# ZKTLabs/zkt-plonk

Measured on AMD Instinct MI355X. Metric: proofs/sec (withdraw, n=2^20), higher is better.
Workload: dtype u32 limbs (256-bit Montgomery); 1 GPU; full prove, WithdrawCircuit INPUTS=8 HEIGHT=64 Poseidon x5 (1019498 gates, 538 Poseidon gadgets), bn254, n=2^20, TABLE_SIZE=1024, 12 public inputs; parallelism=proofs sharded across 1 GPU(s), chained=True, distinct_witnesses=2, witness_on_device=True, table_cached=True, proof_bytes=802

## Files before the change

### zkt-plonk_amd/csrc/msm.hip

```cpp
#include "ctx.hpp"
#include "ec.hpp"
#include "ecx.hpp"
#include "hostec.hpp"
#include "msm.hpp"

#include <algorithm>
#include <functional>
#include <type_traits>
#include <cstdlib>
#include <cstring>

namespace zkt {

template <class C>
__global__ void k_srs_generate(Affine<typename C::Fq>* out, size_t count, Fe<typename C::Fr> tau_mont,
                               Affine<typename C::Fq> g, size_t first) {
    using Q = typename C::Fq;
    using R = typename C::Fr;
    size_t i = (size_t)blockIdx.x * blockDim.x + threadIdx.x;
    if (i >= count) return;
    Fe<R> s = fe_from_mont<R>(fe_from_mont<R>(fe_pow_u64<R>(tau_mont, (uint64_t)(first + i))));
    Xyzz<Q> acc = xyzz_identity<Q>();
    bool started = false;
#pragma unroll 1
// ... 194 lines not shown
    const bool in = threadIdx.x < 256;
    uint32_t incl = in ? mine : 0u;
#pragma unroll
    for (int d = 1; d < 64; d <<= 1) {
        const uint32_t o = __shfl_up(incl, d);
        if ((int)(threadIdx.x & 63) >= d) incl += o;
    }
    __syncthreads();
    if (in && (threadIdx.x & 63) == 63) wsum[threadIdx.x >> 6] = incl;
    __syncthreads();
    uint32_t before = 0;
    for (uint32_t w = 0; w < (threadIdx.x >> 6) && w < 4; ++w) before += wsum[w];
    return before + incl - (in ? mine : 0u);
}

template <class C, int DIG, bool VB = false>
__global__ __launch_bounds__(1024) void k_msm_bin_count(MsmBatch bt, int mont,
                                                        MsmWindows win, uint32_t per_block, uint32_t nb1, uint32_t lb,
                                                        uint32_t* counts) {
    using R = typename C::Fr;
    const uint32_t y = blockIdx.y;
    const Fe<R>* scalars = (const Fe<R>*)bt.scalars[y];
    const size_t n = bt.n[y];
    counts += y * bt.s_bin_offs;
    extern __shared__ uint32_t lds[];
    uint32_t* hist = lds;
    for (uint32_t b = threadIdx.x; b < nb1; b += 1024) hist[b] = 0;
    __syncthreads();
    Fe<R> sc[2];
    bool have[2];
#pragma unroll
    for (int t = 0; t < 2; ++t) {
        const uint32_t k = threadIdx.x + 1024u * t;
        const size_t i = (size_t)blockIdx.x * per_block + k;
        have[t] = k < per_block && i < n;
        if (have[t]) sc[t] = fe_load<R>(scalars + i);
    }
#pragma unroll
    for (int t = 0; t < 2; ++t) {
        if (!have[t]) continue;
        Fe<R> s = sc[t];
        if (VB) {
            if (mont) s = fe_from_mont<R>(s);
        } else if (!mont) {
            s = fe_to_mont<R>(s);
        }
        msm_for_each_digit_sel<R, DIG>(s, win, [&](int w, uint32_t d, uint32_t) {
            if (d) atomicAdd(&hist[(VB ? (uint32_t)w * bt.vb_stride + d : d) >> lb], 1u);
        });
    }
    __syncthreads();
    for (uint32_t b = threadIdx.x; b < nb1; b += 1024) counts[(size_t)b * gridDim.x + blockIdx.x] = hist[b];
}

constexpr int MSM_SCAN_TILE = 4096;
__global__ __launch_bounds__(1024) void k_msm_scan_tiles(uint32_t* counts, uint32_t total, uint32_t* aux, MsmBatch bt) {
    __shared__ uint32_t wsum[16];
    counts += blockIdx.y * bt.s_bin_offs;
    aux += blockIdx.y * bt.s_bin_aux;
    const uint32_t i0 = blockIdx.x * MSM_SCAN_TILE + threadIdx.x * 4;
    uint32_t v[4];
#pragma unroll
    for (int k = 0; k < 4; ++k) v[k] = (i0 + k < total) ? counts[i0 + k] : 0u;
    const uint32_t mine = v[0] + v[1] + v[2] + v[3];
    uint32_t all;
    uint32_t run = block_excl_scan_1024(mine, wsum, &all);
#pragma unroll
    for (int k = 0; k < 4; ++k) {
        if (i0 + k < total) counts[i0 + k] = run;
        run += v[k];
    }
    if (threadIdx.x == 0) aux[blockIdx.x] = all;
}
ZKT_D uint32_t msm_bin_off(const uint32_t* offs, const uint32_t* aux, size_t i, size_t total) {
    return (i < total) ? offs[i] + aux[i / MSM_SCAN_TILE] : aux[(total + MSM_SCAN_TILE - 1) / MSM_SCAN_TILE];
}
__global__ __launch_bounds__(1024) void k_msm_scan_aux(const uint32_t* offs, uint32_t* aux, uint32_t nt, uint32_t nblk,
                                                       uint32_t nb1, uint32_t* bin_start, uint32_t* tile_start,
                                                       uint2* tile_desc, uint32_t acc_threads, uint32_t B, uint32_t lanes_fold,
                                                       MsmBatch bt) {
    __shared__ uint32_t wsum[16];
    const uint32_t y = blockIdx.y;
    offs += y * bt.s_bin_offs;
    aux += y * bt.s_bin_aux;
    bin_start += y * bt.s_bin;
    tile_start += y * bt.s_bin;
    tile_desc += y * bt.s_tile_desc;
    uint32_t* heavy_count = bt.heavy[y];
    uint32_t* params = bt.params[y];
    uint32_t carry = 0;
    for (uint32_t base = 0; base < nt; base += 1024) {
        const uint32_t i = base + threadIdx.x;
        const uint32_t mine = (i < nt) ? aux[i] : 0u;
        uint32_t all;
        const uint32_t ex = block_excl_scan_1024(mine, wsum, &all);
        if (i < nt) aux[i] = carry + ex;
        carry += all;
    }
    if (threadIdx.x == 0) {
        aux[nt] = carry;
        *heavy_count = 0;
        uint32_t lo = 1;
        const uint32_t twice = lanes_fold ? (carry / B) / 11u : 2u * (carry / B);
        while (lo < (uint32_t)MSM_CHUNK_MIN && (lo + 1) * (lo + 1) <= twice) ++lo;
        const uint32_t even = (uint32_t)(((uint64_t)carry + acc_threads - 1) / acc_threads);
        params[0] = even > lo ? even : lo;
        params[1] = carry;
    }
    __syncthreads();
    const size_t total = (size_t)nb1 * nblk;
    uint32_t s = 0, tiles = 0;
    if (threadIdx.x <= nb1) s = msm_bin_off(offs, aux, (size_t)threadIdx.x * nblk, total);
    if (threadIdx.x < nb1) {
        const uint32_t e = msm_bin_off(offs, aux, (size_t)(threadIdx.x + 1) * nblk, total);
        tiles = (e - s + MSM_L2_TILE - 1) / MSM_L2_TILE;
    }
    uint32_t all;
    const uint32_t ex = block_excl_scan_1024(tiles, wsum, &all);
    if (threadIdx.x <= nb1) {
        bin_start[threadIdx.x] = s;
        tile_start[threadIdx.x] = ex;
    }
    if (threadIdx.x < nb1) {
        const uint32_t be = msm_bin_off(offs, aux, (size_t)(threadIdx.x + 1) * nblk, total);
        for (uint32_t k = 0; k < tiles; ++k) {
            const uint32_t ts = s + k * MSM_L2_TILE;
            tile_desc[ex + k] = make_uint2(ts, (ts + MSM_L2_TILE < be) ? ts + MSM_L2_TILE : be);
        }
    }
}

template <class C, class PF, int DIG, bool VB = false>
__global__ __launch_bounds__(1024) void k_msm_bin_scatter(MsmBatch bt, int mont,
                                                          MsmWindows win, uint32_t per_block,
                                                          uint32_t nb1, uint32_t lb, const uint32_t* offs,
                                                          const uint32_t* aux, typename PF::type* pairs) {
    using R = typename C::Fr;
    const uint32_t y = blockIdx.y;
    const Fe<R>* scalars = (const Fe<R>*)bt.scalars[y];
    const size_t n = bt.n[y], base_off = bt.base_off[y], count = bt.tcount[y];
    offs += y * bt.s_bin_offs;
    aux += y * bt.s_bin_aux;
    pairs = reinterpret_cast<typename PF::type*>(reinterpret_cast<char*>(pairs) + y * bt.s_pairs_bytes);
    extern __shared__ uint32_t lds[];
    __shared__ uint32_t wsum[16];
    uint32_t* cursor = lds;
    uint32_t* delta = lds + nb1;
    uint32_t* first = lds + 2 * nb1;
    typename PF::type* stage = (typename PF::type*)(lds + ((3 * nb1 + 3) & ~3u));
    const size_t total = (size_t)nb1 * gridDim.x;
    uint32_t g0 = 0, mine = 0;
    if (threadIdx.x < nb1) {
        const size_t at = (size_t)threadIdx.x * gridDim.x + blockIdx.x;
        g0 = msm_bin_off(offs, aux, at, total);
        mine = msm_bin_off(offs, aux, at + 1, total) - g0;
    }
    uint32_t staged;
    const uint32_t ex = block_excl_scan_1024(mine, wsum, &staged);
    if (threadIdx.x < nb1) {
        cursor[threadIdx.x] = ex;
        first[threadIdx.x] = ex;
        delta[threadIdx.x] = g0 - ex;
    }
    __syncthreads();
    Fe<R> sc[2];
    bool have[2];
#pragma unroll
    for (int t = 0; t < 2; ++t) {
        const uint32_t k = threadIdx.x + 1024u * t;
        const size_t i = (size_t)blockIdx.x * per_block + k;
// ... 15 lines not shown
                const uint32_t key = VB ? (uint32_t)w * bt.vb_stride + d : d;
                const uint32_t at = atomicAdd(&cursor[key >> lb], 1u);
                stage[at] = PF::make(key, VB ? (uint32_t)(base_off + i) : (uint32_t)((size_t)w * count + base_off + i), neg, lb);
            }
        });
    }
    __syncthreads();
    const uint32_t lane = threadIdx.x & 63u;
    for (uint32_t b = threadIdx.x >> 6; b < nb1; b += 16) {
        const uint32_t s0 = first[b], e0 = cursor[b], d = delta[b];
        for (uint32_t j = s0 + lane; j < e0; j += 64) pairs[d + j] = stage[j];
    }
}

struct L2Item {
    uint32_t s, e;
    bool valid;
};
ZKT_D L2Item msm_l2_item(uint32_t item, uint32_t nb1, const uint32_t* tile_start, const uint2* tile_desc) {
    L2Item r;
    r.valid = item < tile_start[nb1];
    r.s = 0; r.e = 0;
    if (!r.valid) return r;
    const uint2 d = tile_desc[item];
    r.s = d.x;
    r.e = d.y;
    return r;
}

template <class PF, int LC>
__global__ __launch_bounds__(256) void k_msm_l2_count(const typename PF::type* pairs, uint32_t nb1, uint32_t lb,
                                                      const uint32_t* tile_start, const uint2* tile_desc, uint32_t* cnt2,
                                                      MsmBatch bt) {
    constexpr uint32_t COLS = 1u << LC;
    {
        const uint32_t y = blockIdx.y;
        pairs = reinterpret_cast<const typename PF::type*>(reinterpret_cast<const char*>(pairs) + y * bt.s_pairs_bytes);
        tile_start += y * bt.s_bin;
        tile_desc += y * bt.s_tile_desc;
        cnt2 += y * bt.s_cnt;
    }
    __shared__ uint32_t hist[COLS];
    const L2Item it = msm_l2_item(blockIdx.x, nb1, tile_start, tile_desc);
    if (!it.valid) return;
#pragma unroll
    for (uint32_t c = threadIdx.x; c < COLS; c += 256) hist[c] = 0;
    __syncthreads();
    const uint32_t cnt = it.e - it.s;
    for (uint32_t base = 0; base < cnt; base += 256u * 8u) {
        typename PF::type v[8];
#pragma unroll
        for (int k = 0; k < 8; ++k) {
            const uint32_t j = base + 256u * k + threadIdx.x;
            if (j < cnt) v[k] = pairs[it.s + j];
        }
#pragma unroll
        for (int k = 0; k < 8; ++k) {
            const uint32_t j = base + 256u * k + threadIdx.x;
            if (j < cnt) atomicAdd(&hist[PF::low(v[k], lb)], 1u);
        }
    }
    __syncthreads();
#pragma unroll
    for (uint32_t c = threadIdx.x; c < COLS; c += 256) cnt2[(size_t)blockIdx.x * COLS + c] = hist[c];
}

template <int LC>
__global__ __launch_bounds__(256) void k_msm_l2_scan(const uint32_t* cnt2, uint32_t* pos2, const uint32_t* bin_start,
                                                     const uint32_t* tile_start, uint32_t B, uint32_t lb,
                                                     uint32_t* chunk_bucket, MsmBatch bt) {
    constexpr uint32_t COLS = 1u << LC, K = COLS / 256u;
    const uint32_t y = blockIdx.y;
    cnt2 += y * bt.s_cnt;
    pos2 += y * bt.s_cnt;
    bin_start += y * bt.s_bin;
    tile_start += y * bt.s_bin;
    chunk_bucket += y * bt.s_chunk;
    uint32_t* offsets = bt.offsets[y];
    const uint32_t chunk = bt.params[y][0];
    const uint32_t b = blockIdx.x;
    const uint32_t t0 = tile_start[b], t1 = tile_start[b + 1];
    uint32_t run[K];
#pragma unroll
    for (uint32_t k = 0; k < K; ++k) run[k] = 0;
    for (uint32_t t = t0; t < t1; ++t) {
#pragma unroll
        for (uint32_t k = 0; k < K; ++k) {
            const size_t at = (size_t)t * COLS + threadIdx.x * K + k;
            pos2[at] = run[k];
            run[k] += cnt2[at];
        }
    }
    uint32_t mine = 0;
#pragma unroll
    for (uint32_t k = 0; k < K; ++k) mine += run[k];
// ... 20 lines not shown
            if (at < 256) {
                big[at][0] = key; big[at][1] = tb; big[at][2] = te;
            } else {
                for (uint32_t t = tb; t < te; ++t) chunk_bucket[t] = key;
            }
        }
    }
    __syncthreads();
    const uint32_t nb = nbig < 256u ? nbig : 256u;
    for (uint32_t e = 0; e < nb; ++e)
        for (uint32_t t = big[e][1] + threadIdx.x; t < big[e][2]; t += 256) chunk_bucket[t] = big[e][0];
    for (uint32_t t = t0; t < t1; ++t) {
#pragma unroll
        for (uint32_t k = 0; k < K; ++k) pos2[(size_t)t * COLS + threadIdx.x * K + k] += first[k];
    }
}

constexpr int MSM_L2S_THREADS = 1024;
constexpr int MSM_L2S_PER = MSM_L2_TILE / MSM_L2S_THREADS;
template <class PF, int LC>
__global__ __launch_bounds__(MSM_L2S_THREADS) void k_msm_l2_scatter(const typename PF::type* pairs, uint32_t nb1, uint32_t lb,
                                                                    const uint32_t* tile_start, const uint2* tile_desc,
                                                                    const uint32_t* cnt2, const uint32_t* pos2,
                                                                    uint32_t* vals, MsmBatch bt) {
    constexpr uint32_t COLS = 1u << LC;
    {
        const uint32_t y = blockIdx.y;
        pairs = reinterpret_cast<const typename PF::type*>(reinterpret_cast<const char*>(pairs) + y * bt.s_pairs_bytes);
        tile_start += y * bt.s_bin;
        tile_desc += y * bt.s_tile_desc;
// ... 445 lines not shown
        }
        st->slice_off = share->slice_off;
        st->total = share->total;
    } else if ((rc = dev_alloc(c, &st->table, (size_t)P.W * count * sizeof(Affine<Q>)))) {
        return rc;
    }
    size_t m = (size_t)P.W * count;
    constexpr size_t NB = MSM_BATCH;
    auto up = [](size_t x) { return (x + 63) & ~(size_t)63; };
    st->strides.s_vals = up(m);
    st->strides.s_pairs_bytes = up(m) * 8;
    if ((rc = dev_alloc(c, (void**)&st->vals2, NB * st->strides.s_vals * 4))) return rc;
    if ((rc = dev_alloc(c, &st->pairs, NB * st->strides.s_pairs_bytes))) return rc;
    const size_t max_blk = (count + P.l1_scalars - 1) / P.l1_scalars;
    st->strides.s_bin_offs = up((size_t)P.nb1 * max_blk + 1);
    st->strides.s_bin_aux = up((size_t)P.nb1 * max_blk / MSM_SCAN_TILE + 4);
    st->strides.s_bin = up((size_t)P.nb1 + 1);
    st->strides.s_tile_desc = up(P.l2_items);
    st->strides.s_cnt = up((size_t)P.l2_items << P.lcols);
    if ((rc = dev_alloc(c, (void**)&st->bin_offs, NB * st->strides.s_bin_offs * 4))) return rc;
    if ((rc = dev_alloc(c, (void**)&st->bin_aux, NB * st->strides.s_bin_aux * 4))) return rc;
    if ((rc = dev_alloc(c, (void**)&st->bin_start, NB * st->strides.s_bin * 4))) return rc;
    if ((rc = dev_alloc(c, (void**)&st->tile_start, NB * st->strides.s_bin * 4))) return rc;
    if ((rc = dev_alloc(c, &st->tile_desc, NB * st->strides.s_tile_desc * 8))) return rc;
    if ((rc = dev_alloc(c, (void**)&st->cnt2, NB * st->strides.s_cnt * 4))) return rc;
    if ((rc = dev_alloc(c, (void**)&st->pos2, NB * st->strides.s_cnt * 4))) return rc;
    if ((rc = msm_scatter_lds_cap<C, false>(c, P.packed, P.dig))) return rc;
    static_assert(MsmState::SLOTS == 11, "per-slot arrays are sized for 11 slots");
    for (int i = 0; i < MsmState::SLOTS; ++i) {
        if ((rc = dev_alloc(c, (void**)&st->offsets[i], (((size_t)P.nb1 << P.lb) + 2) * 4))) return rc;
        if ((rc = dev_alloc(c, (void**)&st->heavy[i], ((size_t)P.keys + 2) * 4))) return rc;
        if ((rc = dev_alloc(c, (void**)&st->params[i], 16))) return rc;
    }
    if ((rc = msm_acc_setup<C>(c, &st->acc_threads, &st->acc_lds))) return rc;
    size_t max_chunks = std::min(m, st->acc_threads) + 1;
    for (int i = 0; i < MsmState::SLOTS; ++i)
// ... 49 lines not shown
}
int msm_table_finish(zkt_ctx* c, void* table, size_t count) {
    if (c->curve == ZKT_CURVE_BN254) return table_finish<Bn254Curve>(c, table, count);
    return table_finish<Bls381Curve>(c, table, count);
}

void msm_release(zkt_ctx* c) {
    if (!c->msm) return;
    MsmState& st = *c->msm;
    (void)hipStreamSynchronize(c->stream);
    if (st.side) (void)hipStreamSynchronize(st.side);
    wire_bases_drop(c);
    for (DevBuf& b : st.wb_scalars) dev_free(c, b.p);
    dev_free(c, st.wb_dig);
    void* ptrs[] = {st.table_borrowed ? nullptr : st.table, st.table2_borrowed ? nullptr : st.table2, st.vals2, st.pairs,
                    st.bin_offs, st.bin_aux, st.bin_start, st.tile_start, st.cnt2, st.pos2, st.chunk_bucket, st.tile_desc};
    for (void* p : ptrs) dev_free(c, p);
    for (int i = 0; i < MsmState::SLOTS; ++i) {
        dev_free(c, st.heavy[i]); dev_free(c, st.offsets[i]); dev_free(c, st.pieces[i]); dev_free(c, st.params[i]);
        dev_free(c, st.buckets[i]); dev_free(c, st.rowcol[i]);
    }
    c->msm.reset();
}

template <class C>
static int srs_load_t(zkt_ctx* c, const void* src, size_t count, bool src_on_device, size_t slice_off = 0, size_t total = 0) {
    using Q = typename C::Fq;
    if (count == 0) return set_err(c, ZKT_ERR_INVALID_ARGUMENT, "empty SRS");
    if (int rf = refuse_if_forked(c, "loading a key")) return rf;
    msm_release(c);
    int rc = msm_setup<C>(c, count);
// ... 100 lines not shown
    hipLaunchKernelGGL((k_msm_weighted_rows<C, TI>), dim3(q + 1, ky), dim3(64), 0, st.side, q1, q2, st.plan.Bw, tb);
    ZKT_HIP(c, hipGetLastError());
    }
    for (int j = 0; j < k; ++j) ZKT_HIP(c, hipEventRecord(st.ev_done[st.tail_wait[j]], st.side));
    return ZKT_OK;
}

template <class C>
static int msm_launch_tails(zkt_ctx* c) {
    bool inl = c->msm->defer_tails || c->msm->count <= MSM_TAIL_INL_MAX;
    if (const char* e = exp_env("ZKT_MSM_TAIL_INL")) inl = atoi(e) != 0;
    return inl ? msm_launch_tails_t<C, true>(c) : msm_launch_tails_t<C, false>(c);
}

struct MsmWork {
    uint32_t *bin_offs, *bin_aux, *bin_start, *tile_start;
    void* tile_desc;
    uint32_t *cnt2, *pos2;
    void* pairs;
    uint32_t *vals, *chunk_bucket;
};

template <class C, bool VB>
static int msm_launch_grouping(zkt_ctx* c, const MsmPlan& P, const MsmWork& wk, const MsmBatch& bt, int mont, size_t n, unsigned ky,
                               size_t acc_threads, bool defer_tails) {
    const uint32_t S = P.l1_scalars;
    const unsigned nblk = (unsigned)((n + S - 1) / S);
    const uint32_t total = P.nb1 * nblk, ntiles = (total + MSM_SCAN_TILE - 1) / MSM_SCAN_TILE;
    const uint2* tile_desc = (const uint2*)wk.tile_desc;
    {
        auto kc = msm_pick_bin_count<C, VB>(P.dig);
        hipLaunchKernelGGL(kc, dim3(nblk, ky), dim3(1024), (size_t)P.nb1 * 4, c->stream, bt, mont, P.win, S, P.nb1, P.lb, wk.bin_offs);
    }
    hipLaunchKernelGGL(k_msm_scan_tiles, dim3(ntiles, ky), dim3(1024), 0, c->stream, wk.bin_offs, total, wk.bin_aux, bt);
    hipLaunchKernelGGL(k_msm_scan_aux, dim3(1, ky), dim3(1024), 0, c->stream, wk.bin_offs, wk.bin_aux, ntiles, nblk, P.nb1,
                       wk.bin_start, wk.tile_start, (uint2*)wk.tile_desc, (uint32_t)acc_threads, P.keys, defer_tails ? 1u : 0u, bt);
    ZKT_HIP(c, hipGetLastError());
    const size_t lds_scatter = (size_t)((3 * P.nb1 + 3) & ~3u) * 4 + (size_t)MSM_L1_CAP * (P.packed ? 4 : 8);
    const uint32_t items = (uint32_t)((size_t)P.W * n / MSM_L2_TILE + P.nb1);
    if (P.packed) {
        auto ks = msm_pick_bin_scatter<C, PairPacked, VB>(P.dig);
        hipLaunchKernelGGL(ks, dim3(nblk, ky), dim3(1024), lds_scatter, c->stream, bt, mont, P.win, S, P.nb1, P.lb, wk.bin_offs,
                           wk.bin_aux, (uint32_t*)wk.pairs);
        ZKT_HIP(c, hipGetLastError());
        hipLaunchKernelGGL((k_msm_l2_count<PairPacked, 8>), dim3(items, ky), dim3(256), 0, c->stream, (const uint32_t*)wk.pairs,
                           P.nb1, P.lb, wk.tile_start, tile_desc, wk.cnt2, bt);
    } else {
        auto ks = msm_pick_bin_scatter<C, PairWide, VB>(P.dig);
        hipLaunchKernelGGL(ks, dim3(nblk, ky), dim3(1024), lds_scatter, c->stream, bt, mont, P.win, S, P.nb1, P.lb, wk.bin_offs,
                           wk.bin_aux, (uint2*)wk.pairs);
        ZKT_HIP(c, hipGetLastError());
        auto kc2 = P.lcols == 8 ? k_msm_l2_count<PairWide, 8> : k_msm_l2_count<PairWide, 10>;
        hipLaunchKernelGGL(kc2, dim3(items, ky), dim3(256), 0, c->stream, (const uint2*)wk.pairs, P.nb1, P.lb, wk.tile_start,
                           tile_desc, wk.cnt2, bt);
    }
    {
        auto ksc = P.lcols == 8 ? k_msm_l2_scan<8> : k_msm_l2_scan<10>;
        hipLaunchKernelGGL(ksc, dim3(P.nb1, ky), dim3(256), 0, c->stream, wk.cnt2, wk.pos2, wk.bin_start, wk.tile_start, P.keys,
                           P.lb, wk.chunk_bucket, bt);
    }
    if (P.packed) {
        hipLaunchKernelGGL((k_msm_l2_scatter<PairPacked, 8>), dim3(items, ky), dim3(MSM_L2S_THREADS), 0, c->stream,
                           (const uint32_t*)wk.pairs, P.nb1, P.lb, wk.tile_start, tile_desc, wk.cnt2, wk.pos2, wk.vals, bt);
    } else {
        auto kss = P.lcols == 8 ? k_msm_l2_scatter<PairWide, 8> : k_msm_l2_scatter<PairWide, 10>;
        hipLaunchKernelGGL(kss, dim3(items, ky), dim3(MSM_L2S_THREADS), 0, c->stream, (const uint2*)wk.pairs, P.nb1, P.lb,
                           wk.tile_start, tile_desc, wk.cnt2, wk.pos2, wk.vals, bt);
    }
    ZKT_HIP(c, hipGetLastError());
    return ZKT_OK;
}

template <class C>
static int msm_launch_accumulate(zkt_ctx* c, const MsmPlan& P, const uint32_t* vals, const uint32_t* chunk_bucket, const MsmBatch& bt,
// ... 26 lines not shown
        const int slot = slots[jj];
        if (j < k && st.pending[slot]) ZKT_HIP(c, hipStreamWaitEvent(c->stream, st.ev_done[slot], 0));
        bt.scalars[j] = d_scalars[jj];
        bt.n[j] = ns[jj];
        bt.base_off[j] = base_offs[jj];
        bt.table[j] = st.tbl_table(tbls[jj]);
        bt.tcount[j] = st.tbl_count(tbls[jj]);
        bt.heavy[j] = st.heavy[slot];
        bt.params[j] = st.params[slot];
        bt.offsets[j] = st.offsets[slot];
        bt.pieces[j] = st.pieces[slot];
        if (j < k) n_max = std::max(n_max, ns[jj]);
    }
    {
    ProfScope prof_all(c, all_lag ? "msm_lag_main" : "msm_main", nullptr, (uint64_t)k);
    const MsmWork wk{st.bin_offs, st.bin_aux, st.bin_start, st.tile_start, st.tile_desc, st.cnt2, st.pos2, st.pairs, st.vals2,
                     st.chunk_bucket};
    if (int rc = msm_launch_grouping<C, false>(c, st.plan, wk, bt, mont, n_max, (unsigned)k, st.acc_threads, st.defer_tails))
        return rc;
    for (int j = 0; j < k; ++j) {
        MsmBatch one = bt;
        one.offsets[0] = bt.offsets[j];
        one.pieces[0] = bt.pieces[j];
        one.params[0] = bt.params[j];
        one.table[0] = bt.table[j];
        {
            ProfScope prof_acc(c, tbls[j] ? "msm_lag_accumulate" : "msm_accumulate");
            if (int rc = msm_launch_accumulate<C>(c, st.plan, st.vals2 + (size_t)j * st.strides.s_vals,
                                                  st.chunk_bucket + (size_t)j * st.strides.s_chunk, one, ns[j], st.acc_threads, st.acc_lds))
                return rc;
        }
// ... 264 lines not shown
    using Q = typename C::Fq;
    Affine<Q> res;
    res.x = fe_zero<Q>();
    res.y = fe_zero<Q>();
    if (n > 0) {
        MsmPlan P;
        int rc = msm_bases_plan(c, n, mont, P);
        if (rc) return rc;
        MsmBasesState* st = nullptr;
        if ((rc = msm_bases_state<C>(c, &st))) return rc;
        const int W = P.W;
        const uint32_t q = (uint32_t)(P.c - 1), q2 = q / 2, q1 = q - q2;
        const uint32_t sums = (1u << q1) + (1u << q2);
        const size_t m = (size_t)W * n;
        const size_t nblk = (n + P.l1_scalars - 1) / P.l1_scalars;
        const size_t total = P.nb1 * nblk, ntiles = (total + MSM_SCAN_TILE - 1) / MSM_SCAN_TILE;
        const size_t max_chunks = std::min(m, st->acc_threads) + 1, l2 = P.l2_items;
        if ((rc = grow(c, st->bases, n * sizeof(Affine<Q>))) || (rc = grow(c, st->vals, m * 4)) ||
            (rc = grow(c, st->pairs, m * (P.packed ? 4 : 8))) || (rc = grow(c, st->bin_offs, (total + 1) * 4)) ||
            (rc = grow(c, st->bin_aux, (ntiles + 4) * 4)) || (rc = grow(c, st->bin_start, ((size_t)P.nb1 + 1) * 4)) ||
            (rc = grow(c, st->tile_start, ((size_t)P.nb1 + 1) * 4)) || (rc = grow(c, st->tile_desc, l2 * 8)) ||
            (rc = grow(c, st->cnt2, (l2 << P.lcols) * 4)) || (rc = grow(c, st->pos2, (l2 << P.lcols) * 4)) ||
            (rc = grow(c, st->chunk_bucket, (max_chunks + 2) * 4)) || (rc = grow(c, st->offsets, (((size_t)P.nb1 << P.lb) + 2) * 4)) ||
            (rc = grow(c, st->heavy, ((size_t)P.keys + 2) * 4)) || (rc = grow(c, st->params, 16)) ||
            (rc = grow(c, st->pieces, (max_chunks + P.keys + 2) * sizeof(XyzzRaw<Q>))) ||
            (rc = grow(c, st->buckets, ((size_t)P.keys + 1) * sizeof(Xyzz<Q>))) ||
            (rc = grow(c, st->rowcol, (size_t)W * sums * sizeof(Xyzz<Q>))))
            return rc;
        if (!scalars_on_device) {
            if ((rc = grow(c, st->scalars, n * 32))) return rc;
            ZKT_HIP(c, hipMemcpyAsync(st->scalars.p, scalars, n * 32, hipMemcpyHostToDevice, c->stream));
            scalars = st->scalars.p;
        }
        ZKT_HIP(c, hipMemcpyAsync(st->bases.p, bases, n * sizeof(Affine<Q>),
                                  bases_on_device ? hipMemcpyDeviceToDevice : hipMemcpyHostToDevice, c->stream));
// ... 1 lines not shown
        ZKT_HIP(c, hipGetLastError());

        MsmBatch bt{};
        for (int j = 0; j < MSM_BATCH; ++j) {
            bt.scalars[j] = scalars;
            bt.n[j] = n;
            bt.base_off[j] = 0;
            bt.table[j] = st->bases.p;
            bt.tcount[j] = n;
            bt.heavy[j] = (uint32_t*)st->heavy.p;
            bt.params[j] = (uint32_t*)st->params.p;
            bt.offsets[j] = (uint32_t*)st->offsets.p;
            bt.pieces[j] = st->pieces.p;
        }
        bt.vb_stride = P.Bw;
        const MsmWork wk{(uint32_t*)st->bin_offs.p, (uint32_t*)st->bin_aux.p, (uint32_t*)st->bin_start.p, (uint32_t*)st->tile_start.p,
                         st->tile_desc.p, (uint32_t*)st->cnt2.p, (uint32_t*)st->pos2.p, st->pairs.p, (uint32_t*)st->vals.p,
                         (uint32_t*)st->chunk_bucket.p};
        {
            ProfScope prof(c, "msm_bases_main");
            if ((rc = msm_launch_grouping<C, true>(c, P, wk, bt, mont, n, 1, st->acc_threads, false)) ||
                (rc = msm_launch_accumulate<C>(c, P, wk.vals, wk.chunk_bucket, bt, n, st->acc_threads, st->acc_lds)))
                return rc;
        }
        {
            ProfScope prof(c, "msm_bases_tail");
            MsmTailBatch tb{};
            for (int j = 0; j < MSM_TAIL_BATCH; ++j) {
                tb.offsets[j] = (const uint32_t*)st->offsets.p;
                tb.params[j] = (const uint32_t*)st->params.p;
                tb.pieces[j] = st->pieces.p;
// ... 145 lines not shown
```

### zkt-plonk_amd/csrc/msm.hpp

```cpp
#pragma once
#include "ctx.hpp"

#include <functional>

namespace zkt {

constexpr int MSM_CHUNK_MIN = 16;
constexpr int MSM_R2_BLOCKS = 1;
constexpr int MSM_MAX_Y = 24;

struct MsmWindows {
    int W;
    uint8_t width[40];
    uint16_t start[40];
};

struct MsmPlan {
    MsmWindows win{};
    int W = 0, c = 0;
    int dig = 0;
    uint32_t Bw = 0;
    uint32_t keys = 0;
    uint32_t lb = 8;
    int lcols = 8;
// ... 2 lines not shown
    uint32_t l1_scalars = 0;
    uint32_t l2_items = 0;
};

constexpr int MSM_BATCH = 3;
struct MsmBatch {
    const void* scalars[MSM_BATCH];
    uint64_t n[MSM_BATCH];
    uint64_t base_off[MSM_BATCH];
    const void* table[MSM_BATCH];
    uint64_t tcount[MSM_BATCH];
    uint32_t* heavy[MSM_BATCH];
    uint32_t* params[MSM_BATCH];
    uint32_t* offsets[MSM_BATCH];
    void* pieces[MSM_BATCH];
    uint64_t s_bin_offs, s_bin_aux, s_bin, s_tile_desc, s_cnt, s_pairs_bytes, s_vals, s_chunk;
    uint32_t vb_stride;
};

constexpr int MSM_TAIL_BATCH = 6;
struct MsmTailBatch {
    const uint32_t* offsets[MSM_TAIL_BATCH];
    const uint32_t* params[MSM_TAIL_BATCH];
    const void* pieces[MSM_TAIL_BATCH];
    void* buckets[MSM_TAIL_BATCH];
    uint32_t* heavy[MSM_TAIL_BATCH];
    void* rowcol[MSM_TAIL_BATCH];
    void* partials[MSM_TAIL_BATCH];
};

constexpr int MSM_HEAVY = 32;
// ... 24 lines not shown
    void* table2 = nullptr;
    size_t count2 = 0;
    int lag_log_n = -1;
    bool lag_failed = false;
    bool table_borrowed = false, table2_borrowed = false;
    WireBases wb;
    DevBuf wb_scalars[3];
    uint64_t* wb_dig = nullptr;
    uint64_t* wb_pin = nullptr;
    const void* tbl_table(int tbl) const { return tbl >= MSM_TBL_WIRE ? wb.table[tbl - MSM_TBL_WIRE] : tbl ? table2 : table; }
    size_t tbl_count(int tbl) const { return tbl >= MSM_TBL_WIRE ? wb.cnt[tbl - MSM_TBL_WIRE] + 2 : tbl ? count2 : count; }
    uint32_t* params[11] = {};
    uint32_t* vals2 = nullptr;
    void* pairs = nullptr;
    uint32_t* bin_offs = nullptr;
    uint32_t* bin_aux = nullptr;
    uint32_t *bin_start = nullptr, *tile_start = nullptr;
    void* tile_desc = nullptr;
    uint32_t *cnt2 = nullptr, *pos2 = nullptr;
    uint32_t* chunk_bucket = nullptr;
    MsmBatch strides{};
    uint32_t* offsets[11] = {};
    void* pieces[11] = {};
    static constexpr int SLOTS = 11;
    void* buckets[SLOTS] = {};
    void* rowcol[SLOTS] = {};
    void* host_result[SLOTS] = {};
    void* host_result_dev[SLOTS] = {};
    size_t acc_lds = 0;
    size_t acc_threads = 196608;
    hipStream_t side = nullptr;
// ... 4 lines not shown
    int n_tail_wait = 0;
    ~MsmState() {
        for (int i = 0; i < SLOTS; ++i) {
            if (host_result[i]) (void)hipHostFree(host_result[i]);
            if (ev_main[i]) (void)hipEventDestroy(ev_main[i]);
            if (ev_done[i]) (void)hipEventDestroy(ev_done[i]);
        }
        if (side) (void)hipStreamDestroy(side);
        if (wb_pin) (void)hipHostFree(wb_pin);
    }
};

struct MsmBasesState {
    DevBuf bases;
    DevBuf scalars;
    DevBuf vals, pairs, bin_offs, bin_aux, bin_start, tile_start, tile_desc, cnt2, pos2, chunk_bucket;
    DevBuf offsets, heavy, params, pieces, buckets, rowcol;
    void* partials = nullptr;
    void* partials_dev = nullptr;
    size_t acc_lds = 0, acc_threads = 0;
    ~MsmBasesState() {
        if (partials) (void)hipHostFree(partials);
    }
};

constexpr size_t MSM_DEFER_MAX = ((size_t)1 << 16) + 64;
constexpr size_t MSM_TAIL_INL_MAX = ((size_t)1 << 18) + 64;

int srs_load(zkt_ctx* c, const void* src, size_t count, bool on_device, size_t slice_off = 0, size_t total = 0);
int srs_generate(zkt_ctx* c, const uint64_t* tau4, size_t count, size_t slice_off = 0, size_t total = 0);
void msm_release(zkt_ctx* c);
// ... 27 lines not shown
```

Baseline: 54.42 proofs/s.

## Fuse MSM bin scans into count kernels via last-arriver tickets

Removes the separate tile-scan and aux-scan kernels after the L1 bin count, as well as the separate L2 per-bin scan kernel. Instead, the last-arriving block of each group (and then the last group overall) does the prefix sums using atomic tickets and agent-scope fences. Tile descriptors now pack a count and a bin index. This cuts several kernel launches and their global round trips per MSM. In exchange it adds atomic and fence overhead, serial scans in the tail block, and correctness risk if tickets are not reset.

```diff
diff --git a/zkt-plonk_amd/csrc/msm.hip b/zkt-plonk_amd/csrc/msm.hip
--- a/zkt-plonk_amd/csrc/msm.hip
+++ b/zkt-plonk_amd/csrc/msm.hip
@@ -232,10 +232,113 @@
     return before + incl - (in ? mine : 0u);
 }
 
+ZKT_D bool msm_last_arriver(uint32_t* ticket, uint32_t expected, uint32_t* flag) {
+    asm volatile("s_waitcnt vmcnt(0)" ::: "memory");
+    __syncthreads();
+    if (threadIdx.x == 0) {
+        __builtin_amdgcn_fence(__ATOMIC_RELEASE, "agent");
+        asm volatile("s_waitcnt vmcnt(0)" ::: "memory");
+        const uint32_t t = __hip_atomic_fetch_add(ticket, 1u, __ATOMIC_RELAXED, __HIP_MEMORY_SCOPE_AGENT);
+        const bool last = t + 1u == expected;
+        if (last) {
+            __hip_atomic_store(ticket, 0u, __ATOMIC_RELAXED, __HIP_MEMORY_SCOPE_AGENT);
+            __builtin_amdgcn_fence(__ATOMIC_ACQUIRE, "agent");
+            asm volatile("s_waitcnt vmcnt(0)" ::: "memory");
+        }
+        *flag = last ? 1u : 0u;
+    }
+    __syncthreads();
+    return *flag != 0u;
+}
+
+static uint32_t msm_l1_group_size(size_t nblk) { return nblk <= 2048 ? 32u : 128u; }
+static size_t msm_l1_groups(size_t nblk) { return (nblk + msm_l1_group_size(nblk) - 1) / msm_l1_group_size(nblk); }
+static size_t msm_l1_groups_max(size_t max_blk) { return (max_blk + 31) / 32; }
+struct MsmL1Scan {
+    uint32_t* gtot;
+    uint32_t* tickets;
+    uint32_t gsize;
+    uint32_t *bin_start, *tile_start;
+    uint2* tile_desc;
+    uint32_t acc_threads, B, lanes_fold;
+};
+ZKT_D uint32_t msm_bin_off(const uint32_t* counts, const uint32_t* gtot, const uint32_t* bin_start, uint32_t nb1, uint32_t nblk,
+                           uint32_t gsize, uint32_t b, uint32_t blk) {
+    if (blk >= nblk) return bin_start[b + 1];
+    return bin_start[b] + gtot[(size_t)(blk / gsize) * nb1 + b] + counts[(size_t)b * nblk + blk];
+}
+constexpr uint32_t MSM_TILE_CNT_BITS = 14;
+
+ZKT_D void msm_l1_finish(uint32_t* counts, uint32_t nb1, const MsmL1Scan& sc, const MsmBatch& bt) {
+    __shared__ uint32_t wsum[16];
+    __shared__ uint32_t flag;
+    const uint32_t y = blockIdx.y, nblk = gridDim.x, G = sc.gsize;
+    const uint32_t ngroups = (nblk + G - 1) / G, group = blockIdx.x / G;
+    const uint32_t g0 = group * G, gcnt = (nblk - g0 < G) ? nblk - g0 : G;
+    uint32_t* tickets = sc.tickets + y * bt.s_tickets;
+    uint32_t* gtot = sc.gtot + y * bt.s_gtot;
+    const uint32_t b = threadIdx.x;
+    if (!msm_last_arriver(tickets + 1 + group, gcnt, &flag)) return;
+    if (b < nb1) {
+        uint32_t* row = counts + (size_t)b * nblk + g0;
+        uint32_t run = 0;
+        for (uint32_t k0 = 0; k0 < gcnt; k0 += 8) {
+            uint32_t v[8];
+#pragma unroll
+            for (uint32_t k = 0; k < 8; ++k) v[k] = (k0 + k < gcnt) ? row[k0 + k] : 0u;
+#pragma unroll
+            for (uint32_t k = 0; k < 8; ++k) {
+                if (k0 + k < gcnt) row[k0 + k] = run;
+                run += v[k];
+            }
+        }
+        gtot[(size_t)group * nb1 + b] = run;
+    }
+    if (!msm_last_arriver(tickets, ngroups, &flag)) return;
+    uint32_t mine = 0;
+    if (b < nb1) {
+        for (uint32_t k0 = 0; k0 < ngroups; k0 += 8) {
+            uint32_t v[8];
+#pragma unroll
+            for (uint32_t k = 0; k < 8; ++k) v[k] = (k0 + k < ngroups) ? gtot[(size_t)(k0 + k) * nb1 + b] : 0u;
+#pragma unroll
+            for (uint32_t k = 0; k < 8; ++k) {
+                if (k0 + k < ngroups) gtot[(size_t)(k0 + k) * nb1 + b] = mine;
+                mine += v[k];
+            }
+        }
+    }
+    uint32_t pairs;
+    const uint32_t s = block_excl_scan_1024(mine, wsum, &pairs);
+    const uint32_t tiles = (mine + MSM_L2_TILE - 1) / MSM_L2_TILE;
+    uint32_t all;
+    const uint32_t ex = block_excl_scan_1024(tiles, wsum, &all);
+    uint32_t* bin_start = sc.bin_start + y * bt.s_bin;
+    uint32_t* tile_start = sc.tile_start + y * bt.s_bin;
+    uint2* tile_desc = sc.tile_desc + y * bt.s_tile_desc;
+    if (b <= nb1) {
+        bin_start[b] = s;
+        tile_start[b] = ex;
+    }
+    for (uint32_t k = 0; k < tiles; ++k) {
+        const uint32_t ts = k * MSM_L2_TILE, left = mine - ts;
+        tile_desc[ex + k] = make_uint2(s + ts, (left < (uint32_t)MSM_L2_TILE ? left : (uint32_t)MSM_L2_TILE) | (b << MSM_TILE_CNT_BITS));
+    }
+    if (threadIdx.x == 0) {
+        *bt.heavy[y] = 0;
+        uint32_t lo = 1;
+        const uint32_t twice = sc.lanes_fold ? (pairs / sc.B) / 11u : 2u * (pairs / sc.B);
+        while (lo < (uint32_t)MSM_CHUNK_MIN && (lo + 1) * (lo + 1) <= twice) ++lo;
+        const uint32_t even = (uint32_t)(((uint64_t)pairs + sc.acc_threads - 1) / sc.acc_threads);
+        bt.params[y][0] = even > lo ? even : lo;
+        bt.params[y][1] = pairs;
+    }
+}
+
 template <class C, int DIG, bool VB = false>
 __global__ __launch_bounds__(1024) void k_msm_bin_count(MsmBatch bt, int mont,
                                                         MsmWindows win, uint32_t per_block, uint32_t nb1, uint32_t lb,
-                                                        uint32_t* counts) {
+                                                        uint32_t* counts, MsmL1Scan sc) {
     using R = typename C::Fr;
     const uint32_t y = blockIdx.y;
     const Fe<R>* scalars = (const Fe<R>*)bt.scalars[y];
@@ -245,19 +348,19 @@
     uint32_t* hist = lds;
     for (uint32_t b = threadIdx.x; b < nb1; b += 1024) hist[b] = 0;
     __syncthreads();
-    Fe<R> sc[2];
+    Fe<R> sc2[2];
     bool have[2];
 #pragma unroll
     for (int t = 0; t < 2; ++t) {
         const uint32_t k = threadIdx.x + 1024u * t;
         const size_t i = (size_t)blockIdx.x * per_block + k;
         have[t] = k < per_block && i < n;
-        if (have[t]) sc[t] = fe_load<R>(scalars + i);
+        if (have[t]) sc2[t] = fe_load<R>(scalars + i);
     }
 #pragma unroll
     for (int t = 0; t < 2; ++t) {
         if (!have[t]) continue;
-        Fe<R> s = sc[t];
+        Fe<R> s = sc2[t];
         if (VB) {
             if (mont) s = fe_from_mont<R>(s);
         } else if (!mont) {
@@ -269,96 +372,22 @@
     }
     __syncthreads();
     for (uint32_t b = threadIdx.x; b < nb1; b += 1024) counts[(size_t)b * gridDim.x + blockIdx.x] = hist[b];
-}
-
-constexpr int MSM_SCAN_TILE = 4096;
-__global__ __launch_bounds__(1024) void k_msm_scan_tiles(uint32_t* counts, uint32_t total, uint32_t* aux, MsmBatch bt) {
-    __shared__ uint32_t wsum[16];
-    counts += blockIdx.y * bt.s_bin_offs;
-    aux += blockIdx.y * bt.s_bin_aux;
-    const uint32_t i0 = blockIdx.x * MSM_SCAN_TILE + threadIdx.x * 4;
-    uint32_t v[4];
-#pragma unroll
-    for (int k = 0; k < 4; ++k) v[k] = (i0 + k < total) ? counts[i0 + k] : 0u;
-    const uint32_t mine = v[0] + v[1] + v[2] + v[3];
-    uint32_t all;
-    uint32_t run = block_excl_scan_1024(mine, wsum, &all);
-#pragma unroll
-    for (int k = 0; k < 4; ++k) {
-        if (i0 + k < total) counts[i0 + k] = run;
-        run += v[k];
-    }
-    if (threadIdx.x == 0) aux[blockIdx.x] = all;
-}
-ZKT_D uint32_t msm_bin_off(const uint32_t* offs, const uint32_t* aux, size_t i, size_t total) {
-    return (i < total) ? offs[i] + aux[i / MSM_SCAN_TILE] : aux[(total + MSM_SCAN_TILE - 1) / MSM_SCAN_TILE];
-}
-__global__ __launch_bounds__(1024) void k_msm_scan_aux(const uint32_t* offs, uint32_t* aux, uint32_t nt, uint32_t nblk,
-                                                       uint32_t nb1, uint32_t* bin_start, uint32_t* tile_start,
-                                                       uint2* tile_desc, uint32_t acc_threads, uint32_t B, uint32_t lanes_fold,
-                                                       MsmBatch bt) {
-    __shared__ uint32_t wsum[16];
-    const uint32_t y = blockIdx.y;
-    offs += y * bt.s_bin_offs;
-    aux += y * bt.s_bin_aux;
-    bin_start += y * bt.s_bin;
-    tile_start += y * bt.s_bin;
-    tile_desc += y * bt.s_tile_desc;
-    uint32_t* heavy_count = bt.heavy[y];
-    uint32_t* params = bt.params[y];
-    uint32_t carry = 0;
-    for (uint32_t base = 0; base < nt; base += 1024) {
-        const uint32_t i = base + threadIdx.x;
-        const uint32_t mine = (i < nt) ? aux[i] : 0u;
-        uint32_t all;
-        const uint32_t ex = block_excl_scan_1024(mine, wsum, &all);
-        if (i < nt) aux[i] = carry + ex;
-        carry += all;
-    }
-    if (threadIdx.x == 0) {
-        aux[nt] = carry;
-        *heavy_count = 0;
-        uint32_t lo = 1;
-        const uint32_t twice = lanes_fold ? (carry / B) / 11u : 2u * (carry / B);
-        while (lo < (uint32_t)MSM_CHUNK_MIN && (lo + 1) * (lo + 1) <= twice) ++lo;
-        const uint32_t even = (uint32_t)(((uint64_t)carry + acc_threads - 1) / acc_threads);
-        params[0] = even > lo ? even : lo;
-        params[1] = carry;
-    }
-    __syncthreads();
-    const size_t total = (size_t)nb1 * nblk;
-    uint32_t s = 0, tiles = 0;
-    if (threadIdx.x <= nb1) s = msm_bin_off(offs, aux, (size_t)threadIdx.x * nblk, total);
-    if (threadIdx.x < nb1) {
-        const uint32_t e = msm_bin_off(offs, aux, (size_t)(threadIdx.x + 1) * nblk, total);
-        tiles = (e - s + MSM_L2_TILE - 1) / MSM_L2_TILE;
-    }
-    uint32_t all;
-    const uint32_t ex = block_excl_scan_1024(tiles, wsum, &all);
-    if (threadIdx.x <= nb1) {
-        bin_start[threadIdx.x] = s;
-        tile_start[threadIdx.x] = ex;
-    }
-    if (threadIdx.x < nb1) {
-        const uint32_t be = msm_bin_off(offs, aux, (size_t)(threadIdx.x + 1) * nblk, total);
-        for (uint32_t k = 0; k < tiles; ++k) {
-            const uint32_t ts = s + k * MSM_L2_TILE;
-            tile_desc[ex + k] = make_uint2(ts, (ts + MSM_L2_TILE < be) ? ts + MSM_L2_TILE : be);
-        }
-    }
+    msm_l1_finish(counts, nb1, sc, bt);
 }
 
 template <class C, class PF, int DIG, bool VB = false>
 __global__ __launch_bounds__(1024) void k_msm_bin_scatter(MsmBatch bt, int mont,
                                                           MsmWindows win, uint32_t per_block,
                                                           uint32_t nb1, uint32_t lb, const uint32_t* offs,
-                                                          const uint32_t* aux, typename PF::type* pairs) {
+                                                          const uint32_t* gtot, const uint32_t* bin_start, uint32_t gsize,
+                                                          typename PF::type* pairs) {
     using R = typename C::Fr;
     const uint32_t y = blockIdx.y;
     const Fe<R>* scalars = (const Fe<R>*)bt.scalars[y];
     const size_t n = bt.n[y], base_off = bt.base_off[y], count = bt.tcount[y];
     offs += y * bt.s_bin_offs;
-    aux += y * bt.s_bin_aux;
+    gtot += y * bt.s_gtot;
+    bin_start += y * bt.s_bin;
     pairs = reinterpret_cast<typename PF::type*>(reinterpret_cast<char*>(pairs) + y * bt.s_pairs_bytes);
     extern __shared__ uint32_t lds[];
     __shared__ uint32_t wsum[16];
@@ -366,12 +395,10 @@
     uint32_t* delta = lds + nb1;
     uint32_t* first = lds + 2 * nb1;
     typename PF::type* stage = (typename PF::type*)(lds + ((3 * nb1 + 3) & ~3u));
-    const size_t total = (size_t)nb1 * gridDim.x;
     uint32_t g0 = 0, mine = 0;
     if (threadIdx.x < nb1) {
-        const size_t at = (size_t)threadIdx.x * gridDim.x + blockIdx.x;
-        g0 = msm_bin_off(offs, aux, at, total);
-        mine = msm_bin_off(offs, aux, at + 1, total) - g0;
+        g0 = msm_bin_off(offs, gtot, bin_start, nb1, gridDim.x, gsize, threadIdx.x, blockIdx.x);
+        mine = msm_bin_off(offs, gtot, bin_start, nb1, gridDim.x, gsize, threadIdx.x, blockIdx.x + 1) - g0;
     }
     uint32_t staged;
     const uint32_t ex = block_excl_scan_1024(mine, wsum, &staged);
@@ -417,71 +444,25 @@
 }
 
 struct L2Item {
-    uint32_t s, e;
+    uint32_t s, e, bin;
     bool valid;
 };
 ZKT_D L2Item msm_l2_item(uint32_t item, uint32_t nb1, const uint32_t* tile_start, const uint2* tile_desc) {
     L2Item r;
     r.valid = item < tile_start[nb1];
-    r.s = 0; r.e = 0;
+    r.s = 0; r.e = 0; r.bin = 0;
     if (!r.valid) return r;
     const uint2 d = tile_desc[item];
     r.s = d.x;
-    r.e = d.y;
+    r.e = d.x + (d.y & ((1u << MSM_TILE_CNT_BITS) - 1u));
+    r.bin = d.y >> MSM_TILE_CNT_BITS;
     return r;
 }
 
-template <class PF, int LC>
-__global__ __launch_bounds__(256) void k_msm_l2_count(const typename PF::type* pairs, uint32_t nb1, uint32_t lb,
-                                                      const uint32_t* tile_start, const uint2* tile_desc, uint32_t* cnt2,
-                                                      MsmBatch bt) {
-    constexpr uint32_t COLS = 1u << LC;
-    {
-        const uint32_t y = blockIdx.y;
-        pairs = reinterpret_cast<const typename PF::type*>(reinterpret_cast<const char*>(pairs) + y * bt.s_pairs_bytes);
-        tile_start += y * bt.s_bin;
-        tile_desc += y * bt.s_tile_desc;
-        cnt2 += y * bt.s_cnt;
-    }
-    __shared__ uint32_t hist[COLS];
-    const L2Item it = msm_l2_item(blockIdx.x, nb1, tile_start, tile_desc);
-    if (!it.valid) return;
-#pragma unroll
-    for (uint32_t c = threadIdx.x; c < COLS; c += 256) hist[c] = 0;
-    __syncthreads();
-    const uint32_t cnt = it.e - it.s;
-    for (uint32_t base = 0; base < cnt; base += 256u * 8u) {
-        typename PF::type v[8];
-#pragma unroll
-        for (int k = 0; k < 8; ++k) {
-            const uint32_t j = base + 256u * k + threadIdx.x;
-            if (j < cnt) v[k] = pairs[it.s + j];
-        }
-#pragma unroll
-        for (int k = 0; k < 8; ++k) {
-            const uint32_t j = base + 256u * k + threadIdx.x;
-            if (j < cnt) atomicAdd(&hist[PF::low(v[k], lb)], 1u);
-        }
-    }
-    __syncthreads();
-#pragma unroll
-    for (uint32_t c = threadIdx.x; c < COLS; c += 256) cnt2[(size_t)blockIdx.x * COLS + c] = hist[c];
-}
-
 template <int LC>
-__global__ __launch_bounds__(256) void k_msm_l2_scan(const uint32_t* cnt2, uint32_t* pos2, const uint32_t* bin_start,
-                                                     const uint32_t* tile_start, uint32_t B, uint32_t lb,
-                                                     uint32_t* chunk_bucket, MsmBatch bt) {
+ZKT_D void msm_l2_scan_bin(uint32_t b, uint32_t* cnt2, uint32_t* pos2, const uint32_t* bin_start, const uint32_t* tile_start,
+                           uint32_t B, uint32_t lb, uint32_t* chunk_bucket, uint32_t* offsets, uint32_t chunk) {
     constexpr uint32_t COLS = 1u << LC, K = COLS / 256u;
-    const uint32_t y = blockIdx.y;
-    cnt2 += y * bt.s_cnt;
-    pos2 += y * bt.s_cnt;
-    bin_start += y * bt.s_bin;
-    tile_start += y * bt.s_bin;
-    chunk_bucket += y * bt.s_chunk;
-    uint32_t* offsets = bt.offsets[y];
-    const uint32_t chunk = bt.params[y][0];
-    const uint32_t b = blockIdx.x;
     const uint32_t t0 = tile_start[b], t1 = tile_start[b + 1];
     uint32_t run[K];
 #pragma unroll
@@ -532,6 +513,58 @@
 #pragma unroll
         for (uint32_t k = 0; k < K; ++k) pos2[(size_t)t * COLS + threadIdx.x * K + k] += first[k];
     }
+}
+
+template <class PF, int LC>
+__global__ __launch_bounds__(256) void k_msm_l2_count(const typename PF::type* pairs, uint32_t nb1, uint32_t lb,
+                                                      const uint32_t* tile_start, const uint2* tile_desc, uint32_t* cnt2,
+                                                      uint32_t* pos2, const uint32_t* bin_start, uint32_t B, uint32_t* chunk_bucket,
+                                                      uint32_t* tickets, MsmBatch bt) {
+    constexpr uint32_t COLS = 1u << LC;
+    const uint32_t y = blockIdx.y;
+    pairs = reinterpret_cast<const typename PF::type*>(reinterpret_cast<const char*>(pairs) + y * bt.s_pairs_bytes);
+    tile_start += y * bt.s_bin;
+    bin_start += y * bt.s_bin;
+    tile_desc += y * bt.s_tile_desc;
+    cnt2 += y * bt.s_cnt;
+    pos2 += y * bt.s_cnt;
+    chunk_bucket += y * bt.s_chunk;
+    tickets += y * bt.s_tickets;
+    uint32_t* offsets = bt.offsets[y];
+    __shared__ uint32_t hist[COLS];
+    __shared__ uint32_t flag;
+    const L2Item it = msm_l2_item(blockIdx.x, nb1, tile_start, tile_desc);
+    if (!it.valid) {
+        const uint32_t ntiles = tile_start[nb1], spare = gridDim.x - ntiles;
+        for (uint32_t b = blockIdx.x - ntiles; b < nb1; b += spare) {
+            if (tile_start[b + 1] != tile_start[b]) continue;
+            const uint32_t at = bin_start[b];
+            for (uint32_t col = threadIdx.x; col < (1u << lb); col += 256) offsets[(b << lb) + col] = at;
+        }
+        return;
+    }
+#pragma unroll
+    for (uint32_t c = threadIdx.x; c < COLS; c += 256) hist[c] = 0;
+    __syncthreads();
+    const uint32_t cnt = it.e - it.s;
+    for (uint32_t base = 0; base < cnt; base += 256u * 8u) {
+        typename PF::type v[8];
+#pragma unroll
+        for (int k = 0; k < 8; ++k) {
+            const uint32_t j = base + 256u * k + threadIdx.x;
+            if (j < cnt) v[k] = pairs[it.s + j];
+        }
+#pragma unroll
+        for (int k = 0; k < 8; ++k) {
+            const uint32_t j = base + 256u * k + threadIdx.x;
+            if (j < cnt) atomicAdd(&hist[PF::low(v[k], lb)], 1u);
+        }
+    }
+    __syncthreads();
+#pragma unroll
+    for (uint32_t c = threadIdx.x; c < COLS; c += 256) cnt2[(size_t)blockIdx.x * COLS + c] = hist[c];
+    if (!msm_last_arriver(tickets + it.bin, tile_start[it.bin + 1] - tile_start[it.bin], &flag)) return;
+    msm_l2_scan_bin<LC>(it.bin, cnt2, pos2, bin_start, tile_start, B, lb, chunk_bucket, offsets, bt.params[y][0]);
 }
 
 constexpr int MSM_L2S_THREADS = 1024;
@@ -1007,12 +1040,16 @@
     if ((rc = dev_alloc(c, &st->pairs, NB * st->strides.s_pairs_bytes))) return rc;
     const size_t max_blk = (count + P.l1_scalars - 1) / P.l1_scalars;
     st->strides.s_bin_offs = up((size_t)P.nb1 * max_blk + 1);
-    st->strides.s_bin_aux = up((size_t)P.nb1 * max_blk / MSM_SCAN_TILE + 4);
+    st->strides.s_gtot = up((size_t)P.nb1 * msm_l1_groups_max(max_blk));
+    st->strides.s_tickets = up(1 + msm_l1_groups_max(max_blk) + (size_t)P.nb1);
     st->strides.s_bin = up((size_t)P.nb1 + 1);
     st->strides.s_tile_desc = up(P.l2_items);
     st->strides.s_cnt = up((size_t)P.l2_items << P.lcols);
     if ((rc = dev_alloc(c, (void**)&st->bin_offs, NB * st->strides.s_bin_offs * 4))) return rc;
-    if ((rc = dev_alloc(c, (void**)&st->bin_aux, NB * st->strides.s_bin_aux * 4))) return rc;
+    if ((rc = dev_alloc(c, (void**)&st->gtot, NB * st->strides.s_gtot * 4))) return rc;
+    if ((rc = dev_alloc(c, (void**)&st->tickets, NB * st->strides.s_tickets * 4))) return rc;
+    ZKT_HIP(c, hipMemsetAsync(st->tickets, 0, NB * st->strides.s_tickets * 4, c->stream));
+    ZKT_HIP(c, hipStreamSynchronize(c->stream));
     if ((rc = dev_alloc(c, (void**)&st->bin_start, NB * st->strides.s_bin * 4))) return rc;
     if ((rc = dev_alloc(c, (void**)&st->tile_start, NB * st->strides.s_bin * 4))) return rc;
     if ((rc = dev_alloc(c, &st->tile_desc, NB * st->strides.s_tile_desc * 8))) return rc;
@@ -1092,7 +1129,7 @@
     for (DevBuf& b : st.wb_scalars) dev_free(c, b.p);
     dev_free(c, st.wb_dig);
     void* ptrs[] = {st.table_borrowed ? nullptr : st.table, st.table2_borrowed ? nullptr : st.table2, st.vals2, st.pairs,
-                    st.bin_offs, st.bin_aux, st.bin_start, st.tile_start, st.cnt2, st.pos2, st.chunk_bucket, st.tile_desc};
+                    st.bin_offs, st.gtot, st.tickets, st.bin_start, st.tile_start, st.cnt2, st.pos2, st.chunk_bucket, st.tile_desc};
     for (void* p : ptrs) dev_free(c, p);
     for (int i = 0; i < MsmState::SLOTS; ++i) {
         dev_free(c, st.heavy[i]); dev_free(c, st.offsets[i]); dev_free(c, st.pieces[i]); dev_free(c, st.params[i]);
@@ -1223,7 +1260,7 @@
 }
 
 struct MsmWork {
-    uint32_t *bin_offs, *bin_aux, *bin_start, *tile_start;
+    uint32_t *bin_offs, *gtot, *tickets, *bin_start, *tile_start;
     void* tile_desc;
     uint32_t *cnt2, *pos2;
     void* pairs;
@@ -1235,38 +1272,34 @@
                                size_t acc_threads, bool defer_tails) {
     const uint32_t S = P.l1_scalars;
     const unsigned nblk = (unsigned)((n + S - 1) / S);
-    const uint32_t total = P.nb1 * nblk, ntiles = (total + MSM_SCAN_TILE - 1) / MSM_SCAN_TILE;
+    const uint32_t gsize = msm_l1_group_size(nblk);
     const uint2* tile_desc = (const uint2*)wk.tile_desc;
+    uint32_t* l2_tickets = wk.tickets + 1 + msm_l1_groups(nblk);
     {
         auto kc = msm_pick_bin_count<C, VB>(P.dig);
-        hipLaunchKernelGGL(kc, dim3(nblk, ky), dim3(1024), (size_t)P.nb1 * 4, c->stream, bt, mont, P.win, S, P.nb1, P.lb, wk.bin_offs);
-    }
-    hipLaunchKernelGGL(k_msm_scan_tiles, dim3(ntiles, ky), dim3(1024), 0, c->stream, wk.bin_offs, total, wk.bin_aux, bt);
-    hipLaunchKernelGGL(k_msm_scan_aux, dim3(1, ky), dim3(1024), 0, c->stream, wk.bin_offs, wk.bin_aux, ntiles, nblk, P.nb1,
-                       wk.bin_start, wk.tile_start, (uint2*)wk.tile_desc, (uint32_t)acc_threads, P.keys, defer_tails ? 1u : 0u, bt);
+        const MsmL1Scan sc{wk.gtot, wk.tickets, gsize, wk.bin_start, wk.tile_start, (uint2*)wk.tile_desc, (uint32_t)acc_threads,
+                           P.keys, defer_tails ? 1u : 0u};
+        hipLaunchKernelGGL(kc, dim3(nblk, ky), dim3(1024), (size_t)P.nb1 * 4, c->stream, bt, mont, P.win, S, P.nb1, P.lb, wk.bin_offs, sc);
+    }
     ZKT_HIP(c, hipGetLastError());
     const size_t lds_scatter = (size_t)((3 * P.nb1 + 3) & ~3u) * 4 + (size_t)MSM_L1_CAP * (P.packed ? 4 : 8);
     const uint32_t items = (uint32_t)((size_t)P.W * n / MSM_L2_TILE + P.nb1);
     if (P.packed) {
         auto ks = msm_pick_bin_scatter<C, PairPacked, VB>(P.dig);
         hipLaunchKernelGGL(ks, dim3(nblk, ky), dim3(1024), lds_scatter, c->stream, bt, mont, P.win, S, P.nb1, P.lb, wk.bin_offs,
-                           wk.bin_aux, (uint32_t*)wk.pairs);
+                           wk.gtot, wk.bin_start, gsize, (uint32_t*)wk.pairs);
         ZKT_HIP(c, hipGetLastError());
         hipLaunchKernelGGL((k_msm_l2_count<PairPacked, 8>), dim3(items, ky), dim3(256), 0, c->stream, (const uint32_t*)wk.pairs,
-                           P.nb1, P.lb, wk.tile_start, tile_desc, wk.cnt2, bt);
+                           P.nb1, P.lb, wk.tile_start, tile_desc, wk.cnt2, wk.pos2, wk.bin_start, P.keys, wk.chunk_bucket,
+                           l2_tickets, bt);
     } else {
         auto ks = msm_pick_bin_scatter<C, PairWide, VB>(P.dig);
         hipLaunchKernelGGL(ks, dim3(nblk, ky), dim3(1024), lds_scatter, c->stream, bt, mont, P.win, S, P.nb1, P.lb, wk.bin_offs,
-                           wk.bin_aux, (uint2*)wk.pairs);
+                           wk.gtot, wk.bin_start, gsize, (uint2*)wk.pairs);
         ZKT_HIP(c, hipGetLastError());
         auto kc2 = P.lcols == 8 ? k_msm_l2_count<PairWide, 8> : k_msm_l2_count<PairWide, 10>;
         hipLaunchKernelGGL(kc2, dim3(items, ky), dim3(256), 0, c->stream, (const uint2*)wk.pairs, P.nb1, P.lb, wk.tile_start,
-                           tile_desc, wk.cnt2, bt);
-    }
-    {
-        auto ksc = P.lcols == 8 ? k_msm_l2_scan<8> : k_msm_l2_scan<10>;
-        hipLaunchKernelGGL(ksc, dim3(P.nb1, ky), dim3(256), 0, c->stream, wk.cnt2, wk.pos2, wk.bin_start, wk.tile_start, P.keys,
-                           P.lb, wk.chunk_bucket, bt);
+                           tile_desc, wk.cnt2, wk.pos2, wk.bin_start, P.keys, wk.chunk_bucket, l2_tickets, bt);
     }
     if (P.packed) {
         hipLaunchKernelGGL((k_msm_l2_scatter<PairPacked, 8>), dim3(items, ky), dim3(MSM_L2S_THREADS), 0, c->stream,
@@ -1323,7 +1356,7 @@
     }
     {
     ProfScope prof_all(c, all_lag ? "msm_lag_main" : "msm_main", nullptr, (uint64_t)k);
-    const MsmWork wk{st.bin_offs, st.bin_aux, st.bin_start, st.tile_start, st.tile_desc, st.cnt2, st.pos2, st.pairs, st.vals2,
+    const MsmWork wk{st.bin_offs, st.gtot, st.tickets, st.bin_start, st.tile_start, st.tile_desc, st.cnt2, st.pos2, st.pairs, st.vals2,
                      st.chunk_bucket};
     if (int rc = msm_launch_grouping<C, false>(c, st.plan, wk, bt, mont, n_max, (unsigned)k, st.acc_threads, st.defer_tails))
         return rc;
@@ -1618,11 +1651,16 @@
         const uint32_t sums = (1u << q1) + (1u << q2);
         const size_t m = (size_t)W * n;
         const size_t nblk = (n + P.l1_scalars - 1) / P.l1_scalars;
-        const size_t total = P.nb1 * nblk, ntiles = (total + MSM_SCAN_TILE - 1) / MSM_SCAN_TILE;
+        const size_t total = P.nb1 * nblk, groups = msm_l1_groups(nblk);
         const size_t max_chunks = std::min(m, st->acc_threads) + 1, l2 = P.l2_items;
+        {
+            const size_t had = st->tickets.bytes;
+            if ((rc = grow(c, st->tickets, (1 + groups + (size_t)P.nb1) * 4))) return rc;
+            if (st->tickets.bytes != had) ZKT_HIP(c, hipMemsetAsync(st->tickets.p, 0, st->tickets.bytes, c->stream));
+        }
         if ((rc = grow(c, st->bases, n * sizeof(Affine<Q>))) || (rc = grow(c, st->vals, m * 4)) ||
             (rc = grow(c, st->pairs, m * (P.packed ? 4 : 8))) || (rc = grow(c, st->bin_offs, (total + 1) * 4)) ||
-            (rc = grow(c, st->bin_aux, (ntiles + 4) * 4)) || (rc = grow(c, st->bin_start, ((size_t)P.nb1 + 1) * 4)) ||
+            (rc = grow(c, st->gtot, groups * P.nb1 * 4)) || (rc = grow(c, st->bin_start, ((size_t)P.nb1 + 1) * 4)) ||
             (rc = grow(c, st->tile_start, ((size_t)P.nb1 + 1) * 4)) || (rc = grow(c, st->tile_desc, l2 * 8)) ||
             (rc = grow(c, st->cnt2, (l2 << P.lcols) * 4)) || (rc = grow(c, st->pos2, (l2 << P.lcols) * 4)) ||
             (rc = grow(c, st->chunk_bucket, (max_chunks + 2) * 4)) || (rc = grow(c, st->offsets, (((size_t)P.nb1 << P.lb) + 2) * 4)) ||
@@ -1654,7 +1692,7 @@
             bt.pieces[j] = st->pieces.p;
         }
         bt.vb_stride = P.Bw;
-        const MsmWork wk{(uint32_t*)st->bin_offs.p, (uint32_t*)st->bin_aux.p, (uint32_t*)st->bin_start.p, (uint32_t*)st->tile_start.p,
+        const MsmWork wk{(uint32_t*)st->bin_offs.p, (uint32_t*)st->gtot.p, (uint32_t*)st->tickets.p, (uint32_t*)st->bin_start.p, (uint32_t*)st->tile_start.p,
                          st->tile_desc.p, (uint32_t*)st->cnt2.p, (uint32_t*)st->pos2.p, st->pairs.p, (uint32_t*)st->vals.p,
                          (uint32_t*)st->chunk_bucket.p};
         {
diff --git a/zkt-plonk_amd/csrc/msm.hpp b/zkt-plonk_amd/csrc/msm.hpp
--- a/zkt-plonk_amd/csrc/msm.hpp
+++ b/zkt-plonk_amd/csrc/msm.hpp
@@ -40,7 +40,7 @@
     uint32_t* params[MSM_BATCH];
     uint32_t* offsets[MSM_BATCH];
     void* pieces[MSM_BATCH];
-    uint64_t s_bin_offs, s_bin_aux, s_bin, s_tile_desc, s_cnt, s_pairs_bytes, s_vals, s_chunk;
+    uint64_t s_bin_offs, s_gtot, s_tickets, s_bin, s_tile_desc, s_cnt, s_pairs_bytes, s_vals, s_chunk;
     uint32_t vb_stride;
 };
 
@@ -95,7 +95,8 @@
     uint32_t* vals2 = nullptr;
     void* pairs = nullptr;
     uint32_t* bin_offs = nullptr;
-    uint32_t* bin_aux = nullptr;
+    uint32_t* gtot = nullptr;
+    uint32_t* tickets = nullptr;
     uint32_t *bin_start = nullptr, *tile_start = nullptr;
     void* tile_desc = nullptr;
     uint32_t *cnt2 = nullptr, *pos2 = nullptr;
@@ -130,7 +131,7 @@
 struct MsmBasesState {
     DevBuf bases;
     DevBuf scalars;
-    DevBuf vals, pairs, bin_offs, bin_aux, bin_start, tile_start, tile_desc, cnt2, pos2, chunk_bucket;
+    DevBuf vals, pairs, bin_offs, gtot, tickets, bin_start, tile_start, tile_desc, cnt2, pos2, chunk_bucket;
     DevBuf offsets, heavy, params, pieces, buckets, rowcol;
     void* partials = nullptr;
     void* partials_dev = nullptr;
```

Result: slower. 51.59 proofs/s (-5.2%).
